# yc-huang/bsdb

Hardware: AMD Instinct MI355X
Metric: index-build keys/s (device-resident), 13B x 13-byte keys; % HBM roofline (higher is better)
Workload: dtype u64

## Files before the change

bsdb_amd/csrc/capi_hist.hip:

```cpp

P1Args key_args(const uint8_t *keys, const uint64_t *offsets, uint64_t blob_bytes, uint32_t key_len, uint64_t n,
                uint64_t seed) {
    P1Args a{};
    a.keys = keys;
    a.offsets = offsets;
    a.blob_bytes = blob_bytes;
    a.key_len = key_len;
    a.n = n;
    a.seed = seed;
    return a;
}

P1Args slice(const P1Args &a0, bool var, uint64_t k0, uint64_t nk, uint64_t blob) {
    P1Args a = a0;
    a.n = nk;
    if (var) {
        a.offsets = a0.offsets + k0;
    } else {
        a.keys = a0.keys + k0 * a0.key_len;
        a.blob_bytes = blob;
    }
    if (a.sig) a.sig = a0.sig + 2 * k0;
    return a;
}
P1Args slice(const P1Args &a, bool var, const KeyRange &r) { return slice(a, var, r.k0, r.nk, r.blob); }

constexpr uint64_t MAX_TILES_PER_LAUNCH = (1ULL << 32) / P1_THREADS - 1;

template <int EPI>
void launch_pass1(const P1Args &a, bool var, uint32_t key_len, uint64_t tiles, hipStream_t s, int frontend) {
    if (tiles > MAX_TILES_PER_LAUNCH) {
        for (uint64_t t0 = 0; t0 < tiles; t0 += MAX_TILES_PER_LAUNCH) {
            const uint64_t nt = std::min(MAX_TILES_PER_LAUNCH, tiles - t0), k0 = t0 * P1_TILE;
            launch_pass1<EPI>(slice(a, var, k0, std::min<uint64_t>(a.n - k0, nt * P1_TILE), a.blob_bytes - k0 * key_len),
                              var, key_len, nt, s, frontend);
        }
        return;
    }
    const dim3 g((uint32_t)tiles), b(P1_THREADS);
    if (var && frontend == 2) {
        k_pass1<SRC_VAR, EPI, 1, 0><<<g, b, 0, s>>>(a);
    } else if (var) {
        k_pass1<SRC_VARSTAGED, EPI, 1, 0><<<g, b, 0, s>>>(a);
    } else if (key_len == 13 && frontend != 1) {
        k_pass1<SRC_DIRECT13, EPI, 4, 13><<<g, b, 0, s>>>(a);
    } else if (key_len == 13) {
        k_pass1<SRC_STAGED13, EPI, 4, 13><<<g, b, 0, s>>>(a);
    } else if (key_len >= 1 && key_len <= 13) {
        k_pass1<SRC_STAGED, EPI, 4, 0><<<g, b, 0, s>>>(a);
    } else if (key_len >= 14 && key_len <= 26) {
        k_pass1<SRC_STAGED, EPI, 2, 0><<<g, b, 0, s>>>(a);
    } else if (key_len >= 27 && key_len <= 52) {
        k_pass1<SRC_STAGED, EPI, 1, 0><<<g, b, 0, s>>>(a);
    } else {
        k_pass1<SRC_FIXED_DIRECT, EPI, 1, 0><<<g, b, 0, s>>>(a);
    }
}

using D13Kernel = void (*)(P1Args, uint64_t);

D13Kernel pass1_kernel(const Pass1Choice &k) {
    const bool seed0 = k.seed0;
    switch (k.kind) {
        case P1Kind::D13: return k_pass1_d13<D13_NT>;
        case P1Kind::D13E:
            return k.key_len == 8    ? (seed0 ? k_pass1_d13e<0, true, 8> : k_pass1_d13e<0, false, 8>)
                   : k.key_len == 12 ? (seed0 ? k_pass1_d13e<0, true, 12> : k_pass1_d13e<0, false, 12>)
                   : k.key_len == 16 ? (seed0 ? k_pass1_d13e<0, true, 16> : k_pass1_d13e<0, false, 16>)
                   : k.variant == 13 ? (seed0 ? k_pass1_d13e<13, true> : k_pass1_d13e<13>)
                                     : (seed0 ? k_pass1_d13e<0, true> : k_pass1_d13e<0>);
        case P1Kind::VARE:
            return k.key_len == 0 ? (seed0 ? k_pass1_vare<false, true> : k_pass1_vare<false>)
                                  : (seed0 ? k_pass1_vare<true, true> : k_pass1_vare<true>);
        case P1Kind::NONE: break;
    }
    return nullptr;
}

constexpr uint64_t FU_MIN_SUPER = 4;

int fused13_impl(bsdb_ctx *c, const uint8_t *keys, uint64_t blob_bytes, uint64_t n, uint64_t seed, uint64_t m,
                 uint32_t *counts, hipStream_t s, uint64_t *done) {
    *done = 0;
    const uint64_t per = (uint64_t)FU_OWNERS * FU_TILE;
    if (c->num_cus != FU_OWNERS || m == 0 || m > (uint64_t)FU_OWNERS * (FU_TCAP - 2)) return BSDB_OK;
    if (blob_bytes < 3) return BSDB_OK;
    const uint64_t nsuper = std::min(n / per, (blob_bytes - 3) / 13 / per);
    if (nsuper < FU_MIN_SUPER) return BSDB_OK;
    if (n / m > 16384) return BSDB_OK;
    static int per_cu = -1;
    if (per_cu < 0 && hipOccupancyMaxActiveBlocksPerMultiprocessor(&per_cu, k_hist13_fused<true>, FU_NT, 0) != hipSuccess)
        per_cu = 0;
    if (per_cu < 1) return BSDB_OK;
    const size_t sync_bytes = FU_SYNC_U64 * sizeof(uint64_t);
    const size_t ring_bytes = (size_t)FU_SLOTS * FU_SLOT_BYTES;
    int rc = c->fu_ring.grow(ring_bytes + sync_bytes);
    if (rc) return rc;
    FusedArgs fa{};
    fa.keys = keys;
    fa.nsuper = nsuper;
    fa.seed = seed;
    fa.mult = (uint32_t)(2 * m);
    fa.m = (uint32_t)m;
    fa.ring = c->fu_ring.as<uint8_t>();
    fa.sync = (uint64_t *)(c->fu_ring.as<uint8_t>() + ring_bytes);
    fa.overflow = c->overflow.as<uint32_t>();
    fa.counts = counts;
    HIP_OK(hipMemsetAsync(fa.sync, 0, sync_bytes, s));
    HIP_OK(hipMemsetAsync(c->overflow.p, 0, sizeof(uint32_t), s));
    ++c->fu_launches;
    {
        ProfScope ps(c, s, 0, nsuper * per);
        if (seed == 0 && !getenv("BSDB_NO_SEED0"))
            k_hist13_fused<true><<<FU_OWNERS, FU_NT, 0, s>>>(fa);
        else
            k_hist13_fused<false><<<FU_OWNERS, FU_NT, 0, s>>>(fa);
    }
    P1Args af = key_args(keys, nullptr, blob_bytes, 13, nsuper * per, seed);
    af.multiplier = 2 * m;
    af.counts = counts;
    af.overflow = c->overflow.as<uint32_t>();
    k_overflow_fallback<SRC_FIXED_DIRECT, 0><<<1024, P1_THREADS, 0, s>>>(af);
    if ((rc = launch_status())) return rc;
    *done = nsuper * per;
    return BSDB_OK;
}

bool fused_wanted(const bsdb_ctx *c) {
    if (c->hist_mode == 3) return true;
    if (c->hist_mode != 0) return false;
    if (c->fused >= 0) return c->fused == 1;
    return false;
}

struct HistOpts {
    uint64_t chunk_keys, span_max;
};
HistOpts hist_opts(const bsdb_ctx *c) { return {c->chunk_keys, c->span_max}; }

HistIn hist_knobs(const bsdb_ctx *c, HistOpts opts) {
    HistIn in;
    in.hist_mode = c->hist_mode, in.frontend = c->frontend, in.d13_variant = c->d13_variant, in.d13_copies = c->d13_copies;
    in.chunk_keys = opts.chunk_keys, in.span_max = opts.span_max;
    in.pipe = c->pipe == 1, in.pipe_chunks = c->pipe_chunks, in.pipe_cus = c->pipe_cus;
    in.no_fixed_window = getenv("BSDB_NO_FIXED_WINDOW") != nullptr;
    in.no_seed0 = getenv("BSDB_NO_SEED0") != nullptr;
    if (const char *v = getenv("BSDB_D13_GRID")) in.d13_grid = atoll(v);
    in.num_cus = c->num_cus;
    return in;
}

int pipe_begin(bsdb_ctx *c, hipStream_t s, hipStream_t *s2) {
    if (!c->p2_stream && hipStreamCreateWithFlags(&c->p2_stream, hipStreamNonBlocking) != hipSuccess) return BSDB_EIO;
    for (auto &e : c->pipe_ev)
        if (!e && hipEventCreateWithFlags(&e, hipEventDisableTiming) != hipSuccess) return BSDB_EIO;
    *s2 = c->p2_stream;
    HIP_OK(hipEventRecord(c->pipe_ev[4], s));
    HIP_OK(hipStreamWaitEvent(*s2, c->pipe_ev[4], 0));
    return BSDB_OK;
}

void region_args(P1Args &a, const HistPlan &p) {
    a.cap = p.cap;
    a.nparts = p.nparts;
    a.nregions = p.nmain;
    a.region0 = 0;
    a.ncopy = p.nmain;
    a.bin_shift = p.bin_shift;
    a.capb = p.capb;
}
P2Layout pass2_layout(const HistPlan &p, uint64_t m, uint32_t *counts) {
    P2Layout L{};
    L.cap = p.cap;
    L.cap_tail = p.cap_tail;
    L.nparts = p.nparts;
    L.nmain = p.nmain;
    L.ntail = p.ntail;
    L.bshift = PART_SHIFT - p.bin_shift;
    L.num_buckets = m;
    L.counts = counts;
    return L;
}

int histogram_impl(bsdb_ctx *c, const uint8_t *keys, const uint64_t *offsets, uint64_t blob_bytes,
                   uint32_t key_len, uint64_t n, uint64_t seed, uint64_t m, uint32_t *counts, HistOpts opts,
                   hipStream_t s) {
    if (n == 0) return BSDB_OK;
    const bool var = offsets != nullptr;
    if (!var && key_len == 13 && fused_wanted(c)) {
        uint64_t done = 0;
        const int rc = fused13_impl(c, keys, blob_bytes, n, seed, m, counts, s, &done);
        if (rc) return rc;
        if (done) return histogram_impl(c, keys + done * 13, nullptr, blob_bytes - done * 13, 13, n - done, seed, m,
                                        counts, opts, s);
    }
    HistIn in = hist_knobs(c, opts);
    in.var = var, in.key_len = key_len, in.n = n, in.m = m, in.blob_bytes = blob_bytes, in.seed0 = seed == 0;
    HistPlan p = pass1_select(in);
    P1Args a = key_args(keys, offsets, blob_bytes, key_len, n, seed);
    a.multiplier = 2 * m;
    a.counts = counts;
    if (p.atomic_mode) {
        ProfScope ps(c, s, 0, n);
        launch_pass1<EPI_ATOMIC>(a, var, key_len, p1_tiles(n), s, c->frontend);
        return launch_status();
    }
    const D13Kernel kern = pass1_kernel(p.k);
    if (kern && hipOccupancyMaxActiveBlocksPerMultiprocessor(&in.wg_per_cu, kern, p.k.nt(), 0) != hipSuccess) in.wg_per_cu = 0;
    size_t total_b = 0;
    if (hipMemGetInfo(&in.free_bytes, &total_b) != hipSuccess) in.free_bytes = 0;
    in.ids_bytes = c->ids.bytes;
    hist_size(in, p);
    int rc;
    if ((rc = c->ids.grow(p.ids_bytes())) || (rc = c->cursor.grow(p.cursor_bytes())) ||
        (rc = c->p2_pref.grow(p.prefix_bytes())))
        return rc;
    hipStream_t s2 = s;
    if (p.pipe && (rc = pipe_begin(c, s, &s2))) return rc;
    a.scratch = c->cursor.as<uint32_t>() + p.nbuf * p.cur_per_buf();
    region_args(a, p);
    P2Layout L = pass2_layout(p, m, counts);
    for (uint64_t i = 0, nspans = p.spans(); i < nspans; ++i) {
        const HistSpan sp = p.span(i);
        const uint32_t b = sp.buf;
        L.ids = a.ids = c->ids.as<uint16_t>() + b * p.ids_per_buf();
        L.cursor = a.cursor = c->cursor.as<uint32_t>() + b * p.cur_per_buf();
        L.overflow = a.overflow = c->overflow.as<uint32_t>() + 4 * b;
        uint64_t *pref = c->p2_pref.as<uint64_t>() + b * (p.cur_per_buf() + 1);
        if (p.pipe && i >= 2) HIP_OK(hipStreamWaitEvent(s, c->pipe_ev[2 + b], 0));
        HIP_OK(hipMemsetAsync(a.cursor, 0, sizeof(uint32_t) * p.cur_per_buf(), s));
        HIP_OK(hipMemsetAsync(a.overflow, 0, sizeof(uint32_t), s));
        for (uint64_t j = 0; j < sp.launches; ++j) {
            const HistLaunch l = p.launch_of(sp, j);
            const P1Args ac = slice(a, var, l.r);
            ProfScope ps(c, s, 0, l.r.nk);
            auto tail = [&] {
                P1Args at = slice(a, var, l.tail);
                at.ids = a.ids + p.set_elems();
                at.cursor = a.cursor + p.nmain * p.nparts;
                at.cap = p.cap_tail;
                at.nregions = p.ntail;
                if (var)
                    k_pass1<SRC_VAR, EPI_PARTITION, 1, 0><<<(uint32_t)l.tail_tiles, P1_THREADS, 0, s>>>(at);
                else
                    launch_pass1<EPI_PARTITION>(at, false, key_len, l.tail_tiles, s, 0);
            };
            if (!kern)
                launch_pass1<EPI_PARTITION>(ac, var, key_len, l.tiles, s, c->frontend);
            else if (l.tiles)
                kern<<<l.grid, p.k.nt(), 0, s>>>(ac, l.tiles);
            if (l.tail.nk) tail();
        }
        if (p.pipe) {
            HIP_OK(hipEventRecord(c->pipe_ev[b], s));
            HIP_OK(hipStreamWaitEvent(s2, c->pipe_ev[b], 0));
        }
        {
            ProfScope ps(c, s2, 1, sp.r.nk);
            k_pass2_plan<<<1, SCAN_THREADS, 0, s2>>>(L, pref);
            k_pass2b<<<sp.p2_grid, P2_THREADS, 0, s2>>>(L, pref);
        }
        const P1Args as = slice(a, var, sp.r);
        if (var) {
            k_overflow_fallback<SRC_VAR, 0><<<1024, P1_THREADS, 0, s2>>>(as);
        } else {
            k_overflow_fallback<SRC_FIXED_DIRECT, 0><<<1024, P1_THREADS, 0, s2>>>(as);
        }
        if (p.pipe) HIP_OK(hipEventRecord(c->pipe_ev[2 + b], s2));
        if ((rc = launch_status())) return rc;
    }
    if (p.pipe) {
        HIP_OK(hipEventRecord(c->pipe_ev[5], s2));
        HIP_OK(hipStreamWaitEvent(s, c->pipe_ev[5], 0));
    }
    return BSDB_OK;
}

int hash_impl(bsdb_ctx *c, const uint8_t *keys, const uint64_t *offsets, uint64_t blob_bytes, uint32_t key_len,
              uint64_t n, uint64_t seed, uint64_t *sig, hipStream_t s) {
    if (n == 0) return BSDB_OK;
    P1Args a = key_args(keys, offsets, blob_bytes, key_len, n, seed);
    a.sig = sig;
    launch_pass1<EPI_SIG>(a, offsets != nullptr, key_len, p1_tiles(n), s, c->frontend);
    return launch_status();
}
```

bsdb_amd/csrc/fused_kernels.hip:

```cpp
#include <hip/hip_runtime.h>
#include <stdint.h>

namespace bsdb {

constexpr int FU_NT = 1024;
constexpr int FU_NW = FU_NT / 64;
constexpr int FU_OWNERS = 256;
constexpr int FU_TILE = FU_NT * 16;
constexpr int FU_HALF = FU_TILE / 2;
constexpr int FU_CAPB = 80;
constexpr int FU_TCAP = 36864;
constexpr int FU_LAG = 5;
constexpr int FU_SLOTS = 8;
static_assert(FU_SLOTS >= 2 * FU_LAG - 3 && (FU_SLOTS & (FU_SLOTS - 1)) == 0, "ring slots");
constexpr int FU_SHARDS = 8;
constexpr int FU_LINE_U64 = 16;
constexpr uint32_t FU_SPIN_MAX = 1u << 21;
constexpr uint32_t FU_HDR_BYTES = FU_OWNERS * 4;
constexpr uint32_t FU_CHUNKS_MAX = FU_OWNERS * (FU_CAPB / 8);
constexpr uint32_t FU_REGION_BYTES = FU_HDR_BYTES + FU_CHUNKS_MAX * 16;
constexpr size_t FU_SLOT_BYTES = (size_t)FU_OWNERS * FU_REGION_BYTES;
constexpr size_t FU_SYNC_U64 = ((size_t)FU_SLOTS * FU_SHARDS + 3) * FU_LINE_U64;
constexpr uint64_t FU_COMMIT = 1, FU_ABORT = 2;

struct FusedArgs {
    const uint8_t *keys;
    uint64_t nsuper;
    uint64_t seed;
    uint32_t mult;
    uint32_t m;
    uint8_t *ring;
    uint64_t *sync;
    uint32_t *overflow;
    uint32_t *counts;
};

typedef __attribute__((address_space(1))) uint64_t fu_gu64;

__device__ __forceinline__ uint64_t fu_load_relaxed(const uint64_t *p) {
    return __hip_atomic_load((fu_gu64 *)p, __ATOMIC_RELAXED, __HIP_MEMORY_SCOPE_AGENT);
}
__device__ __forceinline__ void fu_add_relaxed(uint64_t *p, uint64_t v) {
    (void)__hip_atomic_fetch_add((fu_gu64 *)p, v, __ATOMIC_RELAXED, __HIP_MEMORY_SCOPE_AGENT);
}
__device__ __forceinline__ uint64_t fu_fetch_add_relaxed(uint64_t *p, uint64_t v) {
    return __hip_atomic_fetch_add((fu_gu64 *)p, v, __ATOMIC_RELAXED, __HIP_MEMORY_SCOPE_AGENT);
}
__device__ __forceinline__ void fu_decide(uint64_t *p, uint64_t v) {
    uint64_t expect = 0;
    (void)__hip_atomic_compare_exchange_strong((fu_gu64 *)p, &expect, v, __ATOMIC_RELAXED, __ATOMIC_RELAXED,
                                               __HIP_MEMORY_SCOPE_AGENT);
}

template <bool SEED0>
__global__ __launch_bounds__(FU_NT, 1) void k_hist13_fused(FusedArgs a) {
    constexpr int NT = FU_NT, TILE = FU_TILE, L = 13, CAPB = FU_CAPB;
    const uint64_t seed = SEED0 ? 0ull : a.seed;
    __shared__ uint32_t table[FU_TCAP / 2];
    __shared__ __align__(16) uint16_t bins[2][FU_OWNERS * CAPB];
    __shared__ uint32_t cnt[3][FU_OWNERS];
    __shared__ uint32_t ovf_round[2];
    __shared__ uint64_t red[FU_NW];
    __shared__ uint64_t fin_word;

    const int tid = threadIdx.x;
    const int w = __builtin_amdgcn_readfirstlane(tid >> 6), l = tid & 63;
    const uint32_t p = blockIdx.x;
    const uint32_t mult = a.mult;
    const uint64_t H = 2 * a.nsuper;
    constexpr uint32_t LAG = FU_LAG, SLOTS = FU_SLOTS;
    const uint32_t lo = (uint32_t)(((uint64_t)p * a.m) >> 8);
    const uint32_t hi_b = (uint32_t)min((uint64_t)a.m - 1, (((uint64_t)p + 1) * a.m) >> 8);
    const uint32_t nent = hi_b - lo + 1;

    for (int i = tid; i < FU_TCAP / 2; i += NT) table[i] = 0;
    for (int i = tid; i < 3 * FU_OWNERS; i += NT) (&cnt[0][0])[i] = 0;
    if (tid < 2) ovf_round[tid] = 0;

    const bool owner = l < 16;

    u32x4a S[4][D13_Q];
    const uint32_t lane_off = ((uint32_t)tid * L) & ~3u;
    const uint32_t sh = (((uint32_t)tid * L) & 3u) * 8u;
    auto load_q = [&](auto qc, uint64_t tt) {
        constexpr int q = decltype(qc)::value;
        const uint8_t *tb = a.keys + tt * ((uint64_t)TILE * L);
        const auto rsrc = __builtin_amdgcn_make_buffer_rsrc(const_cast<uint8_t *>(tb), 0, TILE * L + 16, 0x00020000);
#pragma unroll
        for (int j = 0; j < D13_Q; ++j) {
            const auto v = __builtin_amdgcn_raw_buffer_load_b128(rsrc, lane_off, (q * D13_Q + j) * NT * L, 2);
            S[q][j] = u32x4a{v[0], v[1], v[2], v[3]};
        }
    };
    auto hash_q = [&](auto qc, uint32_t *cn, uint32_t bsel) {
        constexpr int q = decltype(qc)::value;
        uint32_t b[D13_Q], o[D13_Q], r[D13_Q];
#pragma unroll
        for (int j = 0; j < D13_Q; ++j)
            b[j] = spooky13_bucket_owner(S[q][j].x, S[q][j].y, S[q][j].z, S[q][j].w, sh, seed, mult, o[j]);
#pragma unroll
        for (int j = 0; j < D13_Q; ++j) r[j] = atomicAdd(&cn[o[j]], 1u);
#pragma unroll
        for (int j = 0; j < D13_Q; ++j) {
            const uint32_t slot = __umul24(o[j], (uint32_t)CAPB) + min(r[j], (uint32_t)CAPB - 1u);
            __builtin_assume(slot < (uint32_t)(FU_OWNERS * CAPB));
            bins[bsel][slot] = (uint16_t)b[j];
        }
    };

    uint32_t o_cnt = 0, o_off = 0, w_off = 0;
    auto write_out = [&](uint64_t y) {
        const uint32_t buf = (uint32_t)(y & 1);
        const uint32_t slot = (uint32_t)(y % SLOTS);
        const auto rsrc = __builtin_amdgcn_make_buffer_rsrc(
            a.ring + (size_t)slot * FU_SLOT_BYTES + (size_t)p * FU_REGION_BYTES, 0, FU_REGION_BYTES, 0x00020000);
        if (owner) {
            const uint32_t hv = (o_off << 16) | o_cnt;
            __builtin_amdgcn_raw_buffer_store_b32(hv, rsrc, 4u * ((uint32_t)w * 16 + (uint32_t)l), 0, 16);
        }
        const uint32_t nch = owner ? (o_cnt + 7) >> 3 : 0;
        const uint32_t st = o_off - w_off;
        const uint32_t total = __builtin_amdgcn_readlane(st + nch, 15);
        for (uint32_t i0 = 0; i0 < total; i0 += 64) {
            const uint32_t i = i0 + l;
            int j = 0;
#pragma unroll
            for (int step = 8; step >= 1; step >>= 1) {
                const uint32_t s_try = __shfl(st, j + step, 64);
                if (s_try <= i) j += step;
            }
            const uint32_t k = i - __shfl(st, j, 64);
            const uint32_t d = (uint32_t)w * 16 + (uint32_t)j;
            if (i < total) {
                const uint4 v = *reinterpret_cast<const uint4 *>(&bins[buf][d * CAPB + 8 * k]);
                __builtin_amdgcn_raw_buffer_store_b128(u32x4{v.x, v.y, v.z, v.w}, rsrc,
                                                       FU_HDR_BYTES + 16u * (w_off + i), 0, 16);
            }
        }
    };
    auto plan_round = [&](uint32_t *cn) -> bool {
        uint32_t c4[4], n4[4], s = 0;
        bool ovf = false;
#pragma unroll
        for (int e = 0; e < 4; ++e) {
            c4[e] = cn[4 * l + e];
            ovf |= c4[e] > (uint32_t)CAPB;
            c4[e] = min(c4[e], (uint32_t)CAPB);
            n4[e] = (c4[e] + 7) >> 3;
            s += n4[e];
        }
        uint32_t x = s;
#pragma unroll
        for (int d = 1; d < 64; d <<= 1) {
            const uint32_t yv = __shfl_up(x, d, 64);
            if (l >= d) x += yv;
        }
        const uint32_t ex = x - s;
        const int src = 4 * w + (l >> 2);
        const uint32_t e = (uint32_t)l & 3;
        const uint32_t pre = __shfl(ex, src, 64);
        const uint32_t c0 = __shfl(c4[0], src, 64), c1 = __shfl(c4[1], src, 64), c2 = __shfl(c4[2], src, 64),
                       c3 = __shfl(c4[3], src, 64);
        const uint32_t n0 = (c0 + 7) >> 3, n1 = (c1 + 7) >> 3, n2 = (c2 + 7) >> 3;
        o_cnt = e == 0 ? c0 : e == 1 ? c1 : e == 2 ? c2 : c3;
        o_off = pre + (e > 0 ? n0 : 0) + (e > 1 ? n1 : 0) + (e > 2 ? n2 : 0);
        w_off = __builtin_amdgcn_readfirstlane(o_off);
        return ovf;
    };

    const uint32_t cprod = (uint32_t)tid >> 2, csub = (uint32_t)tid & 3;
    u32x4 cv[2];
    uint32_t hdr = 0;
    uint32_t hdr_c = 0;
    uint64_t poll = 0;
    bool dead = false;
    uint32_t consumed = 0;
    uint64_t *const pub = a.sync;
    uint64_t *const fin = a.sync + (size_t)FU_SLOTS * FU_SHARDS * FU_LINE_U64;
    uint64_t *const abort_w = fin + FU_LINE_U64;
    uint64_t *const decide = abort_w + FU_LINE_U64;
    auto region_rsrc = [&](uint64_t y) {
        const uint32_t slot = (uint32_t)(y % SLOTS);
        return __builtin_amdgcn_make_buffer_rsrc(a.ring + (size_t)slot * FU_SLOT_BYTES, 0, (uint32_t)FU_SLOT_BYTES,
                                                 0x00020000);
    };
    auto issue_poll = [&](uint64_t y) {
        const uint32_t slot = (uint32_t)(y % SLOTS);
        uint64_t v = 0;
        if (l < FU_SHARDS) v = fu_load_relaxed(pub + ((size_t)slot * FU_SHARDS + l) * FU_LINE_U64);
        poll = v;
    };
    auto poll_sum = [&]() -> uint64_t {
        uint64_t v = poll;
        v += __shfl_xor(v, 1, 64);
        v += __shfl_xor(v, 2, 64);
        v += __shfl_xor(v, 4, 64);
        return __builtin_amdgcn_readfirstlane((uint32_t)v) | ((uint64_t)__builtin_amdgcn_readfirstlane((uint32_t)(v >> 32)) << 32);
    };
    bool any_ovf = false;
    auto wait_round = [&](uint64_t y) {
        const uint32_t expect = (uint32_t)(FU_OWNERS * (y / SLOTS + 1));
        uint64_t v = poll_sum();
        uint32_t spins = 0;
        while (!dead && (uint32_t)v != expect) {
            __builtin_amdgcn_s_sleep(2);
            if (++spins > FU_SPIN_MAX || fu_load_relaxed(abort_w) != 0) {
                dead = true;
                if (l == 0) fu_add_relaxed(abort_w, 1);
                break;
            }
            issue_poll(y);
            v = poll_sum();
        }
        any_ovf |= (v >> 32) != 0;
    };
    auto load_hdr = [&](uint64_t y) {
        hdr = __builtin_amdgcn_raw_buffer_load_b32(region_rsrc(y), cprod * FU_REGION_BYTES + 4u * p, 0, 16);
    };
    auto chunk_off = [&](uint32_t k) { return cprod * FU_REGION_BYTES + FU_HDR_BYTES + 16u * ((hdr_c >> 16) + k); };
    auto consume_load = [&](uint64_t y) {
        hdr_c = hdr;
        const auto rsrc = region_rsrc(y);
#pragma unroll
        for (int i = 0; i < 2; ++i) {
            const auto v = __builtin_amdgcn_raw_buffer_load_b128(rsrc, chunk_off(csub + 4 * i), 0, 16);
            cv[i] = u32x4{v[0], v[1], v[2], v[3]};
        }
    };
    auto add_chunk = [&](const u32x4 &v, uint32_t chunk, uint32_t c) {
#pragma unroll
        for (int e = 0; e < 8; ++e) {
            const uint32_t pos = 8 * chunk + e;
            const uint32_t wv = e < 2 ? v.x : e < 4 ? v.y : e < 6 ? v.z : v.w;
            const uint32_t id = (e & 1) ? wv >> 16 : wv & 0xFFFFu;
            if (pos < c) {
                const uint32_t off = min((id - lo) & 0xFFFFu, (uint32_t)FU_TCAP - 1);
                atomicAdd(&table[off >> 1], 1u << ((off & 1) << 4));
                ++consumed;
            }
        }
    };
    auto consume_add = [&](uint64_t y) {
        const uint32_t c = min(hdr_c & 0xFFFFu, (uint32_t)CAPB);
        add_chunk(cv[0], csub, c);
        add_chunk(cv[1], csub + 4, c);
        const bool far = csub < 2 && c > 8 * (csub + 8);
        if (__any(far)) {
            const auto v = __builtin_amdgcn_raw_buffer_load_b128(region_rsrc(y), chunk_off(csub + 8), 0, 16);
            if (far) add_chunk(u32x4{v[0], v[1], v[2], v[3]}, csub + 8, c);
        }
    };

    uint32_t h3_next = 0;
    auto iter = [&](auto qc, uint64_t h, uint64_t next_t) {
        constexpr int QA = decltype(qc)::value;
        const int64_t yc = (int64_t)h - LAG, yh = yc + 1, yp = yc + 2;
        const uint32_t h3 = h3_next;
        h3_next = h3 == 2 ? 0 : h3 + 1;
        if (h + 1 < H && tid < FU_OWNERS) cnt[h3_next][tid] = 0;
        if (yc >= 0) consume_load((uint64_t)yc);
        if (yh >= 0 && (uint64_t)yh < H) {
            wait_round((uint64_t)yh);
            load_hdr((uint64_t)yh);
        }
        if (yp >= 0 && (uint64_t)yp < H) issue_poll((uint64_t)yp);
        if (h >= 1 && h - 1 < H) write_out(h - 1);
        asm volatile("" ::: "memory");
        if constexpr (QA >= 0) {
            uint32_t *const cn = cnt[h3];
            const uint32_t bsel = (uint32_t)(h & 1);
            hash_q(std::integral_constant<int, QA>{}, cn, bsel);
            load_q(std::integral_constant<int, QA>{}, next_t);
            hash_q(std::integral_constant<int, QA + 1>{}, cn, bsel);
            load_q(std::integral_constant<int, QA + 1>{}, next_t);
        }
        if (yc >= 0 && !dead) consume_add((uint64_t)yc);
        if constexpr (QA >= 0)
            asm volatile("s_waitcnt vmcnt(8)" ::: "memory");
        else
            asm volatile("s_waitcnt vmcnt(0)" ::: "memory");
        __syncthreads();
        if (h < H) {
            const bool ovf = plan_round(cnt[h3]);
            if (ovf) ovf_round[h & 1] = 1;
        }
        if (h >= 1 && h - 1 < H && tid == 0) {
            const uint32_t pb = (uint32_t)((h - 1) & 1);
            const uint64_t ov = ovf_round[pb];
            ovf_round[pb] = 0;
            fu_add_relaxed(pub + ((size_t)((h - 1) % SLOTS) * FU_SHARDS + (p & (FU_SHARDS - 1))) * FU_LINE_U64,
                           1ull + (ov << 32));
        }
    };

    const uint64_t t0 = p;
    load_q(std::integral_constant<int, 0>{}, t0);
    load_q(std::integral_constant<int, 1>{}, t0);
    load_q(std::integral_constant<int, 2>{}, t0);
    load_q(std::integral_constant<int, 3>{}, t0);
    __syncthreads();
    for (uint64_t k = 0; k < a.nsuper; ++k) {
        const uint64_t nt = k + 1 < a.nsuper ? (k + 1) * FU_OWNERS + p : t0;
        iter(std::integral_constant<int, 0>{}, 2 * k, nt);
        iter(std::integral_constant<int, 2>{}, 2 * k + 1, nt);
    }
    for (uint64_t h = H; h < H + LAG; ++h) iter(std::integral_constant<int, -1>{}, h, t0);

    uint64_t tsum = 0;
    for (int i = tid; i < FU_TCAP / 2; i += NT) tsum += (table[i] & 0xFFFFu) + (table[i] >> 16);
    uint64_t diff = (uint64_t)consumed - tsum;
#pragma unroll
    for (int d = 1; d < 64; d <<= 1) diff += __shfl_xor(diff, d, 64);
    if (l == 0) red[w] = diff;
    const int any_dead = __syncthreads_or(dead ? 1 : 0);
    if (tid == 0) {
        uint64_t dsum = 0;
        for (int i = 0; i < FU_NW; ++i) dsum += red[i];
        const bool bad = dsum != 0 || any_dead || any_ovf || fu_load_relaxed(abort_w) != 0;
        const uint64_t now = fu_fetch_add_relaxed(fin, 1ull + ((uint64_t)bad << 32)) + 1ull + ((uint64_t)bad << 32);
        if ((uint32_t)now == (uint32_t)gridDim.x) fu_decide(decide, (now >> 32) ? FU_ABORT : FU_COMMIT);
        uint64_t d = fu_load_relaxed(decide);
        uint32_t spins = 0;
        while (d == 0) {
            __builtin_amdgcn_s_sleep(2);
            if (++spins > FU_SPIN_MAX || fu_load_relaxed(abort_w) != 0) {
                fu_add_relaxed(abort_w, 1);
                fu_decide(decide, FU_ABORT);
            }
            d = fu_load_relaxed(decide);
        }
        fin_word = d;
        if (d == FU_ABORT) atomicOr(a.overflow, 1u);
        if (fu_load_relaxed(abort_w) != 0 && p == 0) atomicAdd(a.overflow + 3, 1u);
    }
    __syncthreads();
    if (fin_word != FU_COMMIT) return;
    for (uint32_t i = tid; i < nent; i += NT) {
        const uint32_t v = (table[i >> 1] >> ((i & 1) << 4)) & 0xFFFFu;
        if (v) atomicAdd(a.counts + lo + i, v);
    }
}

}
```

Baseline: 316.2 billion.

## Replace variable-length ring exchange with fixed 128-byte bins and global spill

Each owner bin in the inter-block exchange ring becomes a fixed 64-entry line padded with a sentinel id, so the per-round planning scan, headers and chunk-offset search are gone. Consumers load two fixed chunks per thread and skip pad entries. Entries beyond 64 per bin are written to a per-block global spill buffer and added to the global counts at the end, replacing the per-round overflow flag. The cost is that the full fixed-size line is always written and read, bins are re-padded after each write-out, and if the spill capacity is exceeded the fused path aborts.

```diff
diff --git a/bsdb_amd/csrc/capi_hist.hip b/bsdb_amd/csrc/capi_hist.hip
--- a/bsdb_amd/csrc/capi_hist.hip
+++ b/bsdb_amd/csrc/capi_hist.hip
@@ -94,8 +94,10 @@
     if (per_cu < 1) return BSDB_OK;
     const size_t sync_bytes = FU_SYNC_U64 * sizeof(uint64_t);
     const size_t ring_bytes = (size_t)FU_SLOTS * FU_SLOT_BYTES;
-    int rc = c->fu_ring.grow(ring_bytes + sync_bytes);
+    int rc = c->fu_ring.grow(ring_bytes + sync_bytes + FU_SPILL_BYTES);
     if (rc) return rc;
+    uint32_t spill_cap = FU_SPILL_CAP;
+    if (const char *v = getenv("BSDB_FU_SPILL_MAX")) spill_cap = (uint32_t)std::min<uint64_t>(strtoull(v, nullptr, 10), FU_SPILL_CAP);
     FusedArgs fa{};
     fa.keys = keys;
     fa.nsuper = nsuper;
@@ -104,6 +106,8 @@
     fa.m = (uint32_t)m;
     fa.ring = c->fu_ring.as<uint8_t>();
     fa.sync = (uint64_t *)(c->fu_ring.as<uint8_t>() + ring_bytes);
+    fa.spill = (uint32_t *)(c->fu_ring.as<uint8_t>() + ring_bytes + sync_bytes);
+    fa.spill_cap = spill_cap;
     fa.overflow = c->overflow.as<uint32_t>();
     fa.counts = counts;
     HIP_OK(hipMemsetAsync(fa.sync, 0, sync_bytes, s));
diff --git a/bsdb_amd/csrc/fused_kernels.hip b/bsdb_amd/csrc/fused_kernels.hip
--- a/bsdb_amd/csrc/fused_kernels.hip
+++ b/bsdb_amd/csrc/fused_kernels.hip
@@ -8,7 +8,9 @@
 constexpr int FU_OWNERS = 256;
 constexpr int FU_TILE = FU_NT * 16;
 constexpr int FU_HALF = FU_TILE / 2;
-constexpr int FU_CAPB = 80;
+constexpr int FU_CAPB = 64;
+constexpr uint32_t FU_ID_PAD = 0xFFFFu;
+constexpr uint32_t FU_SPILL_CAP = 4096;
 constexpr int FU_TCAP = 36864;
 constexpr int FU_LAG = 5;
 constexpr int FU_SLOTS = 8;
@@ -16,10 +18,11 @@
 constexpr int FU_SHARDS = 8;
 constexpr int FU_LINE_U64 = 16;
 constexpr uint32_t FU_SPIN_MAX = 1u << 21;
-constexpr uint32_t FU_HDR_BYTES = FU_OWNERS * 4;
-constexpr uint32_t FU_CHUNKS_MAX = FU_OWNERS * (FU_CAPB / 8);
-constexpr uint32_t FU_REGION_BYTES = FU_HDR_BYTES + FU_CHUNKS_MAX * 16;
-constexpr size_t FU_SLOT_BYTES = (size_t)FU_OWNERS * FU_REGION_BYTES;
+constexpr uint32_t FU_LINE_BYTES = FU_CAPB * 2;
+static_assert(FU_LINE_BYTES == 128 && FU_TCAP <= (int)FU_ID_PAD, "one line per bin; the pad is no id");
+constexpr uint32_t FU_ROW_BYTES = FU_OWNERS * FU_LINE_BYTES;
+constexpr size_t FU_SLOT_BYTES = (size_t)FU_OWNERS * FU_ROW_BYTES;
+constexpr size_t FU_SPILL_BYTES = (size_t)FU_OWNERS * FU_SPILL_CAP * sizeof(uint32_t);
 constexpr size_t FU_SYNC_U64 = ((size_t)FU_SLOTS * FU_SHARDS + 3) * FU_LINE_U64;
 constexpr uint64_t FU_COMMIT = 1, FU_ABORT = 2;
 
@@ -31,6 +34,8 @@
     uint32_t m;
     uint8_t *ring;
     uint64_t *sync;
+    uint32_t *spill;
+    uint32_t spill_cap;
     uint32_t *overflow;
     uint32_t *counts;
 };
@@ -45,6 +50,13 @@
 }
 __device__ __forceinline__ uint64_t fu_fetch_add_relaxed(uint64_t *p, uint64_t v) {
     return __hip_atomic_fetch_add((fu_gu64 *)p, v, __ATOMIC_RELAXED, __HIP_MEMORY_SCOPE_AGENT);
+}
+typedef __attribute__((address_space(1))) uint32_t fu_gu32;
+__device__ __forceinline__ void fu_store_relaxed(uint32_t *p, uint32_t v) {
+    __hip_atomic_store((fu_gu32 *)p, v, __ATOMIC_RELAXED, __HIP_MEMORY_SCOPE_AGENT);
+}
+__device__ __forceinline__ uint32_t fu_load_relaxed(const uint32_t *p) {
+    return __hip_atomic_load((fu_gu32 *)p, __ATOMIC_RELAXED, __HIP_MEMORY_SCOPE_AGENT);
 }
 __device__ __forceinline__ void fu_decide(uint64_t *p, uint64_t v) {
     uint64_t expect = 0;
@@ -59,7 +71,7 @@
     __shared__ uint32_t table[FU_TCAP / 2];
     __shared__ __align__(16) uint16_t bins[2][FU_OWNERS * CAPB];
     __shared__ uint32_t cnt[3][FU_OWNERS];
-    __shared__ uint32_t ovf_round[2];
+    __shared__ uint32_t spill_n;
     __shared__ uint64_t red[FU_NW];
     __shared__ uint64_t fin_word;
 
@@ -75,9 +87,11 @@
 
     for (int i = tid; i < FU_TCAP / 2; i += NT) table[i] = 0;
     for (int i = tid; i < 3 * FU_OWNERS; i += NT) (&cnt[0][0])[i] = 0;
-    if (tid < 2) ovf_round[tid] = 0;
-
-    const bool owner = l < 16;
+    for (int i = tid; i < FU_OWNERS * CAPB; i += NT)
+        reinterpret_cast<uint32_t *>(&bins[0][0])[i] = FU_ID_PAD | (FU_ID_PAD << 16);
+    if (tid == 0) spill_n = 0;
+    const uint32_t spill_cap = min(a.spill_cap, FU_SPILL_CAP);
+    uint32_t *const spill = a.spill + (size_t)p * FU_SPILL_CAP;
 
     u32x4a S[4][D13_Q];
     const uint32_t lane_off = ((uint32_t)tid * L) & ~3u;
@@ -104,74 +118,33 @@
         for (int j = 0; j < D13_Q; ++j) {
             const uint32_t slot = __umul24(o[j], (uint32_t)CAPB) + min(r[j], (uint32_t)CAPB - 1u);
             __builtin_assume(slot < (uint32_t)(FU_OWNERS * CAPB));
-            bins[bsel][slot] = (uint16_t)b[j];
-        }
-    };
-
-    uint32_t o_cnt = 0, o_off = 0, w_off = 0;
+            if (r[j] < (uint32_t)CAPB) {
+                bins[bsel][slot] = (uint16_t)(b[j] - (__umul24(o[j], a.m) >> 8));
+            } else {
+                const uint32_t s = atomicAdd(&spill_n, 1u);
+                if (s < spill_cap) fu_store_relaxed(spill + s, b[j]);
+            }
+        }
+    };
+
     auto write_out = [&](uint64_t y) {
         const uint32_t buf = (uint32_t)(y & 1);
         const uint32_t slot = (uint32_t)(y % SLOTS);
-        const auto rsrc = __builtin_amdgcn_make_buffer_rsrc(
-            a.ring + (size_t)slot * FU_SLOT_BYTES + (size_t)p * FU_REGION_BYTES, 0, FU_REGION_BYTES, 0x00020000);
-        if (owner) {
-            const uint32_t hv = (o_off << 16) | o_cnt;
-            __builtin_amdgcn_raw_buffer_store_b32(hv, rsrc, 4u * ((uint32_t)w * 16 + (uint32_t)l), 0, 16);
-        }
-        const uint32_t nch = owner ? (o_cnt + 7) >> 3 : 0;
-        const uint32_t st = o_off - w_off;
-        const uint32_t total = __builtin_amdgcn_readlane(st + nch, 15);
-        for (uint32_t i0 = 0; i0 < total; i0 += 64) {
-            const uint32_t i = i0 + l;
-            int j = 0;
-#pragma unroll
-            for (int step = 8; step >= 1; step >>= 1) {
-                const uint32_t s_try = __shfl(st, j + step, 64);
-                if (s_try <= i) j += step;
-            }
-            const uint32_t k = i - __shfl(st, j, 64);
-            const uint32_t d = (uint32_t)w * 16 + (uint32_t)j;
-            if (i < total) {
-                const uint4 v = *reinterpret_cast<const uint4 *>(&bins[buf][d * CAPB + 8 * k]);
-                __builtin_amdgcn_raw_buffer_store_b128(u32x4{v.x, v.y, v.z, v.w}, rsrc,
-                                                       FU_HDR_BYTES + 16u * (w_off + i), 0, 16);
-            }
-        }
-    };
-    auto plan_round = [&](uint32_t *cn) -> bool {
-        uint32_t c4[4], n4[4], s = 0;
-        bool ovf = false;
-#pragma unroll
-        for (int e = 0; e < 4; ++e) {
-            c4[e] = cn[4 * l + e];
-            ovf |= c4[e] > (uint32_t)CAPB;
-            c4[e] = min(c4[e], (uint32_t)CAPB);
-            n4[e] = (c4[e] + 7) >> 3;
-            s += n4[e];
-        }
-        uint32_t x = s;
-#pragma unroll
-        for (int d = 1; d < 64; d <<= 1) {
-            const uint32_t yv = __shfl_up(x, d, 64);
-            if (l >= d) x += yv;
-        }
-        const uint32_t ex = x - s;
-        const int src = 4 * w + (l >> 2);
-        const uint32_t e = (uint32_t)l & 3;
-        const uint32_t pre = __shfl(ex, src, 64);
-        const uint32_t c0 = __shfl(c4[0], src, 64), c1 = __shfl(c4[1], src, 64), c2 = __shfl(c4[2], src, 64),
-                       c3 = __shfl(c4[3], src, 64);
-        const uint32_t n0 = (c0 + 7) >> 3, n1 = (c1 + 7) >> 3, n2 = (c2 + 7) >> 3;
-        o_cnt = e == 0 ? c0 : e == 1 ? c1 : e == 2 ? c2 : c3;
-        o_off = pre + (e > 0 ? n0 : 0) + (e > 1 ? n1 : 0) + (e > 2 ? n2 : 0);
-        w_off = __builtin_amdgcn_readfirstlane(o_off);
-        return ovf;
-    };
-
-    const uint32_t cprod = (uint32_t)tid >> 2, csub = (uint32_t)tid & 3;
+        const auto rsrc = __builtin_amdgcn_make_buffer_rsrc(a.ring + (size_t)slot * FU_SLOT_BYTES, 0,
+                                                            (uint32_t)FU_SLOT_BYTES, 0x00020000);
+#pragma unroll
+        for (int rep = 0; rep < 2; ++rep) {
+            const uint32_t i = (uint32_t)tid + (uint32_t)rep * NT;
+            const uint32_t d = i >> 3, k = i & 7;
+            uint4 *const chunk = reinterpret_cast<uint4 *>(&bins[buf][8 * i]);
+            const uint4 v = *chunk;
+            *chunk = uint4{~0u, ~0u, ~0u, ~0u};
+            __builtin_amdgcn_raw_buffer_store_b128(u32x4{v.x, v.y, v.z, v.w}, rsrc,
+                                                   (d * FU_OWNERS + p) * FU_LINE_BYTES + 16u * k, 0, 16);
+        }
+    };
+
     u32x4 cv[2];
-    uint32_t hdr = 0;
-    uint32_t hdr_c = 0;
     uint64_t poll = 0;
     bool dead = false;
     uint32_t consumed = 0;
@@ -214,41 +187,30 @@
         }
         any_ovf |= (v >> 32) != 0;
     };
-    auto load_hdr = [&](uint64_t y) {
-        hdr = __builtin_amdgcn_raw_buffer_load_b32(region_rsrc(y), cprod * FU_REGION_BYTES + 4u * p, 0, 16);
-    };
-    auto chunk_off = [&](uint32_t k) { return cprod * FU_REGION_BYTES + FU_HDR_BYTES + 16u * ((hdr_c >> 16) + k); };
     auto consume_load = [&](uint64_t y) {
-        hdr_c = hdr;
         const auto rsrc = region_rsrc(y);
 #pragma unroll
         for (int i = 0; i < 2; ++i) {
-            const auto v = __builtin_amdgcn_raw_buffer_load_b128(rsrc, chunk_off(csub + 4 * i), 0, 16);
+            const auto v = __builtin_amdgcn_raw_buffer_load_b128(
+                rsrc, p * FU_ROW_BYTES + 16u * ((uint32_t)tid + (uint32_t)i * NT), 0, 16);
             cv[i] = u32x4{v[0], v[1], v[2], v[3]};
         }
     };
-    auto add_chunk = [&](const u32x4 &v, uint32_t chunk, uint32_t c) {
+    auto add_chunk = [&](const u32x4 &v) {
 #pragma unroll
         for (int e = 0; e < 8; ++e) {
-            const uint32_t pos = 8 * chunk + e;
             const uint32_t wv = e < 2 ? v.x : e < 4 ? v.y : e < 6 ? v.z : v.w;
             const uint32_t id = (e & 1) ? wv >> 16 : wv & 0xFFFFu;
-            if (pos < c) {
-                const uint32_t off = min((id - lo) & 0xFFFFu, (uint32_t)FU_TCAP - 1);
+            if (id != FU_ID_PAD) {
+                const uint32_t off = min(id, (uint32_t)FU_TCAP - 1);
                 atomicAdd(&table[off >> 1], 1u << ((off & 1) << 4));
                 ++consumed;
             }
         }
     };
-    auto consume_add = [&](uint64_t y) {
-        const uint32_t c = min(hdr_c & 0xFFFFu, (uint32_t)CAPB);
-        add_chunk(cv[0], csub, c);
-        add_chunk(cv[1], csub + 4, c);
-        const bool far = csub < 2 && c > 8 * (csub + 8);
-        if (__any(far)) {
-            const auto v = __builtin_amdgcn_raw_buffer_load_b128(region_rsrc(y), chunk_off(csub + 8), 0, 16);
-            if (far) add_chunk(u32x4{v[0], v[1], v[2], v[3]}, csub + 8, c);
-        }
+    auto consume_add = [&]() {
+        add_chunk(cv[0]);
+        add_chunk(cv[1]);
     };
 
     uint32_t h3_next = 0;
@@ -259,10 +221,7 @@
         h3_next = h3 == 2 ? 0 : h3 + 1;
         if (h + 1 < H && tid < FU_OWNERS) cnt[h3_next][tid] = 0;
         if (yc >= 0) consume_load((uint64_t)yc);
-        if (yh >= 0 && (uint64_t)yh < H) {
-            wait_round((uint64_t)yh);
-            load_hdr((uint64_t)yh);
-        }
+        if (yh >= 0 && (uint64_t)yh < H) wait_round((uint64_t)yh);
         if (yp >= 0 && (uint64_t)yp < H) issue_poll((uint64_t)yp);
         if (h >= 1 && h - 1 < H) write_out(h - 1);
         asm volatile("" ::: "memory");
@@ -274,20 +233,14 @@
             hash_q(std::integral_constant<int, QA + 1>{}, cn, bsel);
             load_q(std::integral_constant<int, QA + 1>{}, next_t);
         }
-        if (yc >= 0 && !dead) consume_add((uint64_t)yc);
+        if (yc >= 0 && !dead) consume_add();
         if constexpr (QA >= 0)
             asm volatile("s_waitcnt vmcnt(8)" ::: "memory");
         else
             asm volatile("s_waitcnt vmcnt(0)" ::: "memory");
         __syncthreads();
-        if (h < H) {
-            const bool ovf = plan_round(cnt[h3]);
-            if (ovf) ovf_round[h & 1] = 1;
-        }
         if (h >= 1 && h - 1 < H && tid == 0) {
-            const uint32_t pb = (uint32_t)((h - 1) & 1);
-            const uint64_t ov = ovf_round[pb];
-            ovf_round[pb] = 0;
+            const uint64_t ov = spill_n > spill_cap;
             fu_add_relaxed(pub + ((size_t)((h - 1) % SLOTS) * FU_SHARDS + (p & (FU_SHARDS - 1))) * FU_LINE_U64,
                            1ull + (ov << 32));
         }
@@ -316,7 +269,7 @@
     if (tid == 0) {
         uint64_t dsum = 0;
         for (int i = 0; i < FU_NW; ++i) dsum += red[i];
-        const bool bad = dsum != 0 || any_dead || any_ovf || fu_load_relaxed(abort_w) != 0;
+        const bool bad = dsum != 0 || any_dead || any_ovf || spill_n > spill_cap || fu_load_relaxed(abort_w) != 0;
         const uint64_t now = fu_fetch_add_relaxed(fin, 1ull + ((uint64_t)bad << 32)) + 1ull + ((uint64_t)bad << 32);
         if ((uint32_t)now == (uint32_t)gridDim.x) fu_decide(decide, (now >> 32) ? FU_ABORT : FU_COMMIT);
         uint64_t d = fu_load_relaxed(decide);
@@ -339,6 +292,11 @@
         const uint32_t v = (table[i >> 1] >> ((i & 1) << 4)) & 0xFFFFu;
         if (v) atomicAdd(a.counts + lo + i, v);
     }
-}
-
-}
+    const uint32_t nspill = min(spill_n, spill_cap);
+    for (uint32_t i = tid; i < nspill; i += NT) {
+        const uint32_t b = fu_load_relaxed(spill + i);
+        if (b < a.m) atomicAdd(a.counts + b, 1u);
+    }
+}
+
+}
```

After: 316.3 billion, median of 2. No clear change (+0.0%).
